# huakunyang/SummerTTS

Hardware: AMD Instinct MI355X
Metric: audio samples/sec (acoustic model + vocoder, phoneme ids -> int16 PCM on host), single_speaker_fast-shaped synthetic blob (higher is better)
Workload: dtype f32 (decoder trunk convs AND the reverse flow's WaveNet convs (wn_flow.hip, one-utterance calls): fp32 operands as 2 fp16 terms = 22-23 of their 24 mantissa bits, 3 fp16 MFMA products per fp32 product, f32 accumulation -- measured error in `parity`, same tolerance as the exact-fp32 leg; batches addi

## Files before the change

### include/summertts_hip.h

```cpp
#ifndef SUMMERTTS_HIP_H_
#define SUMMERTTS_HIP_H_

#include <stdint.h>

#ifdef __cplusplus
extern "C" {
#endif

typedef struct sts_engine sts_engine;

enum {
    STS_OK = 0,
    STS_EINVAL = -1,
    STS_EMODEL = -2,
    STS_EDEVICE = -3,
    STS_ESTATE = -4
};

int sts_create(const float* blob, int64_t blob_bytes, int device, sts_engine** out);
void sts_destroy(sts_engine* e);

int sts_speaker_num(const sts_engine* e);

typedef struct sts_model_info {
// ... 133 lines not shown

enum { STS_DBG_ATTN_BLOCK_MIN_WGS = 1,
       STS_DBG_TAIL_FUSED = 14 ,
       STS_DBG_UPS_ROWPH = 15 ,
       STS_DBG_CHAIN_STREAMS = 13 ,
       STS_DBG_H2P = 11 ,
       STS_DBG_H2P_TILE = 12 ,
       STS_DBG_MEMO_CLEAR = 10 ,
       STS_DBG_PCM_DIRECT = 9 ,
       STS_DBG_DDS_TAIL = 8 ,
       STS_DBG_ATTN_REG = 7 ,
       STS_DBG_LAUNCH_AHEAD = 6 ,
       STS_DBG_FLOW_FUSED = 5  };
enum { STS_DBG_STREAM_RETRY_STEP = 16, STS_DBG_STREAM_DIRECT = 17 };
enum { STS_DBG_POISON = 18 };
int sts_debug_set(sts_engine* e, int key, int value);

typedef struct sts_profile {
    float ms_text_encoder, ms_duration, ms_flow, ms_decoder, ms_total_device;
    float ms_decoder_mfma;
    int32_t decoder_mfma_launches;
    double flops_text_encoder, flops_duration, flops_flow, flops_decoder;
    double flops_decoder_mfma;
    double bytes_decoder_min;
    int64_t frames, samples, phonemes;
    double flops_decoder_mfma_executed;
    double bytes_text_encoder, bytes_duration, bytes_flow;
    float ms_sync_wait_host;
    double flops_decoder_bf16_issued;
    int64_t conv_math_fallbacks;
// ... 112 lines not shown
```

### summertts_amd/csrc/capi.hip

```cpp
#include <stdlib.h>
#include <string.h>

#include <algorithm>
#include <new>
#include <string>
#include <vector>

#include "engine.hpp"
#include "eq_stream.hpp"
#include "join_stream.hpp"
#include "loud_stream.hpp"

using namespace sts;

struct sts_engine { Engine eng; };

static thread_local std::string g_err;
static int set_err(int code, const std::string& s) { g_err = s; return code; }

extern "C" {

const char* sts_last_error(void) { return g_err.c_str(); }
void sts_free(void* p) { free(p); }

// ... 657 lines not shown
        case STS_DBG_ATTN_BLOCK_MIN_WGS: if (value < 1) return set_err(STS_EINVAL, "threshold must be >= 1"); e->eng.attn_block_min_wgs = value; return STS_OK;
        case STS_DBG_FLOW_FUSED: e->eng.flow_fused = value != 0; return STS_OK;
        case STS_DBG_LAUNCH_AHEAD: if (value < 0 || value > 2) return set_err(STS_EINVAL, "launch_ahead must be 0, 1 or 2"); if ((value == 2) != (e->eng.launch_ahead == 2)) { e->eng.seen_tf_.clear(); e->eng.seen_order_.clear(); } e->eng.launch_ahead = value; return STS_OK;
        case STS_DBG_H2P: e->eng.h2p = value < 0 ? 0 : (value > 4 ? 4 : value); return STS_OK;
        case STS_DBG_H2P_TILE: e->eng.h2p_tile = value; return STS_OK;
        case STS_DBG_CHAIN_STREAMS: e->eng.chain_streams_dbg = value; return STS_OK;
        case STS_DBG_TAIL_FUSED: e->eng.tail_fused = value != 0; return STS_OK;
        case STS_DBG_UPS_ROWPH: e->eng.ups_rowph = value != 0; return STS_OK;
        case STS_DBG_MEMO_CLEAR: e->eng.seen_tf_.clear(); e->eng.seen_order_.clear(); return STS_OK;
        case STS_DBG_ATTN_REG: e->eng.attn_reg = value != 0; return STS_OK;
        case STS_DBG_DDS_TAIL: e->eng.dds_tail = value != 0; return STS_OK;
        case STS_DBG_PCM_DIRECT: e->eng.pcm_direct = value != 0; return STS_OK;
        case STS_DBG_STREAM_RETRY_STEP: e->eng.stream_retry_step = value < 0 ? -1 : value; return STS_OK;
        case STS_DBG_STREAM_DIRECT: e->eng.stream_direct = value != 0; return STS_OK;
        case STS_DBG_POISON: e->eng.poison = (unsigned)value; return STS_OK;
        default: return set_err(STS_EINVAL, "unknown debug key");
    }
}
int sts_set_host_pcm(sts_engine* e, int enable) { if (!e) return set_err(STS_EINVAL, "null engine"); e->eng.host_pcm = enable != 0; return STS_OK; }
int sts_set_profiling(sts_engine* e, int enable) { if (!e) return set_err(STS_EINVAL, "null engine"); e->eng.profiling = enable == 2 ? 2 : (enable != 0 ? 1 : 0); return STS_OK; }

int sts_abi_version(void) { return STS_ABI_VERSION; }

int sts_set_output_rate(sts_engine* e, int32_t rate) {
    if (!e) return set_err(STS_EINVAL, "null engine");
    const int rc = e->eng.set_output_rate(rate);
    return rc == STS_OK ? STS_OK : set_err(rc, e->eng.error());
}
int sts_get_output_rate(const sts_engine* e) {
    if (!e) return set_err(STS_EINVAL, "null engine");
// ... 833 lines not shown
```

### summertts_amd/csrc/engine.hip

```cpp
#include "run_ctx.hpp"
#include <time.h>
#include "knobs.hpp"
#include "../../include/tts_logger.h"

#include <algorithm>
#include <chrono>
#include <math.h>
#include <stdlib.h>
#include <string.h>
#include <thread>

namespace sts {

Engine::~Engine() {
    if (stream) (void)hipStreamSynchronize(stream);
    free_model(model);
    if (arenaT_.base) (void)hipFree(arenaT_.base);
    if (arenaF_.base) (void)hipFree(arenaF_.base);
    if (pinned_) (void)hipHostFree(pinned_);
    if (pinned_pcm_) (void)hipHostFree(pinned_pcm_);
    if (d_rs_table) (void)hipFree(d_rs_table);
    if (loud_host_) (void)hipHostFree(loud_host_);
    if (lim_host_) (void)hipHostFree(lim_host_);
    if (d_eq_) (void)hipFree(d_eq_);
// ... 929 lines not shown
    size_t regA = 0, regB = 0;
    { int S = 1; for (int i = 0; i < M.n_up; i++) { S *= M.up_rate[i]; stage_elems[i] = (size_t)(3 + 4 * M.n_resk) * M.ups[i].Cout * Wcap * S;
          if (i & 1) { if (stage_elems[i] > regB) regB = stage_elems[i]; } else { if (stage_elems[i] > regA) regA = stage_elems[i]; } } }
    const long Lsb = c.Lsb = Wcap * upS + B;
    const int sbC = c.sbC = M.conv_post.Cout;
    bool use_ff = flow_fused && conv_mode == 0 && conv_math == 3 && !M.cp.empty() && wnH > 0;
    for (size_t i = 0; i < M.cp.size() && use_ff; i++)
        use_ff = M.cp[i].ff.ok && M.cp[i].wn.H == wnH && M.cp[i].wn.n == c.wnL && M.cp[i].ff.G == M.cp[0].ff.G && M.cp[i].wn.in[0].k == M.cp[0].wn.in[0].k;
    if (use_ff) {
        long tiles = 0;
        if (B == 1) tiles = (Ftot + 31) / 32;
        else for (int b = 0; b < B; b++) tiles += (p_lenF[b] + 31) / 32;
        use_ff = tiles * M.cp[0].ff.G <= 256;
    }
    c.use_ff = use_ff; c.ffG = use_ff ? M.cp[0].ff.G : 0;
    BufF& bf = c.bf;
    const OutChain& oc = c.oc;
    c.Ocap = oc.run[OS_RESAMPLE] ? out_count((long long)Wcap * hop) + B : (long long)Wcap * hop;
    if (c.join) c.Ocap = oc.run[OS_RESAMPLE] ? out_count(c.FJ * hop) + 1 : c.FJ * hop;
    const long long jwin = ss && c.join ? c.js.window_frames() * hop : c.FJ * hop;
    if (ss && c.join) c.Ocap = oc.run[OS_RESAMPLE] ? out_count(jwin) + 4 : jwin;
    if (ss && oc.run[OS_LIMIT] && oc.run[OS_RESAMPLE]) c.Ocap += B;
    pcm_in_host_ = pcm_direct && host_pcm && !ss && B == 1 && !record_taps && pinned_pcm_dev_ && (size_t)c.Ocap * 2 + 256 <= pinned_pcm_cap_ &&
                   (size_t)c.Ocap * 2 <= ((size_t)4 << 20);
    auto layoutF = [&](Arena& A) {
        A.used = 0;
        for (int q = 0; q < 2; q++) {
            bf.ff_h[q] = A.get<float>(use_ff ? (size_t)wnH * Ftot : 1);
            bf.ff_part[q] = A.get<float>(use_ff ? (size_t)c.ffG * wnH * Ftot : 1);
            bf.ff_macc[q] = A.get<float>(use_ff ? (size_t)c.ffG * (C / 2) * Ftot : 1);
// ... 105 lines not shown
            const DWn& w = cp.wn;
            const DFlowFused& ff = cp.ff;
            const int x0h = cp.flipped ? 1 : 0, x1h = 1 - x0h;
            if (pend_set >= 0 && pend_half != x0h) { finish_half(pend_half, pend_set); pend_set = -1; }
            if (w.has_cond) conv(w.cond, bt.g, lvB, bt.cond_wn, lvB, ConvOpt());
            (void)conv_args(cp.pre, nullptr, lv1, nullptr, lv1, ConvOpt(), nullptr);
            for (int l = 0; l < w.n; l++) {
                ConvOpt og; og.epi = EPI_GATE;
                (void)conv_args(w.in[l], nullptr, lv1, nullptr, lv1, og, nullptr);
                ConvOpt orr; orr.epi = EPI_RESSKIP;
                (void)conv_args(w.rs[l], nullptr, lv1, nullptr, lv1, orr, nullptr);
                FlowLayerArgs A;
                memset(&A, 0, sizeof(A));
                A.seg = lv1.seg; A.B = B; A.max_len = maxF; A.tot = Ftot;
                A.H = w.H; A.half = half; A.G = G; A.Cg = ff.Cg; A.k = w.in[l].k; A.halo = (w.in[l].k - 1) / 2;
                A.layer = l;
                if (l == 0) {
                    A.x0 = cur[x0h]; A.x0_ld = Ftot;
                    if (pend_set >= 0) {
                        A.pend = bf.ff_macc[pend_set]; A.pend_n = G; A.pend_stride = (long)hF;
                        A.x0_out = cur[x0h] == home[x0h] ? alt[x0h] : home[x0h]; A.x0_out_ld = Ftot;
                    }
                    A.w_pre = cp.pre.wh2; A.b_pre = cp.pre.bias; A.s_pre = cp.pre.h2_scale;
                    A.w_gate = ff.gate0; A.s_gate = ff.gate0_scale;
                } else {
                    A.h_in = bf.ff_h[(l - 1) & 1]; A.part_in = bf.ff_part[(l - 1) & 1]; A.part_n = G;
                    A.w_gate = w.in[l].wh2; A.s_gate = w.in[l].h2_scale;
                }
                A.part_stride = (long)((size_t)w.H * Ftot);
                A.h_out = bf.ff_h[l & 1]; A.part_out = bf.ff_part[l & 1];
                A.macc = bf.ff_macc[cs]; A.macc_stride = (long)hF; A.macc_init = l == 0;
// ... 523 lines not shown
```

### summertts_amd/csrc/engine.hpp

```cpp
#pragma once
#include <hip/hip_runtime.h>

#include <deque>
#include <map>
#include <unordered_map>
#include <string>
#include <vector>

#include "../../include/summertts_hip.h"
#include "kernels.hpp"
#include "model.hpp"

namespace sts {

struct Arena {
    char* base = nullptr; size_t cap = 0, used = 0; bool measuring = false;
    void* alloc(size_t bytes) {
        size_t a = (used + 255) & ~(size_t)255;
        used = a + bytes;
        if (measuring) return nullptr;
        return base + a;
    }
    template <typename T> T* get(size_t count) { return (T*)alloc(count * sizeof(T)); }
};
// ... 98 lines not shown
    long ahead_misses = 0;
    static constexpr size_t kMemoEntries = 1024;
    std::unordered_map<unsigned long long, long> seen_tf_; std::deque<unsigned long long> seen_order_;
    bool polite_wait = false;
    struct WaitEst { double us = 0.0; long phonemes = 0; };
    WaitEst wait_est_[2][24];
    void nap_before_wait(int which, long phonemes);
    void note_wait(int which, long phonemes, double waited_us, bool was_ready_at_wake);
    int final_sync(long phonemes);
    int ups_rowph = 1;
    int tail_fused = 1;
    int chain_streams_dbg = -1;
    int h2p = 1;
    int h2p_tile = -1;
    int flow_fused = 1;
    int stream_retry_step = -1;
    int stream_direct = 0;
    unsigned poison = 0;
    int64_t poison_bytes_ = 0;
    hipStream_t stream = nullptr;

private:
    int fail(int code, const std::string& msg) { err_ = msg; return code; }
    bool ensure(Arena& a, size_t bytes);
    bool ensure_pinned(size_t bytes);
    void poison_arena(const Arena& a);
    void poison_host16(void* p, size_t samples);
    void poison_host32(void* p, size_t words);
    ConvArgs conv_args(const DConv& c, const float* x, const Lvl& lin, float* y, const Lvl& lout, const ConvOpt& o, double* flops);
    void conv(const DConv& c, const float* x, const Lvl& lin, float* y, const Lvl& lout, const ConvOpt& o);
// ... 60 lines not shown
```

### summertts_amd/csrc/kernels.hpp

```cpp
#pragma once
#include <hip/hip_runtime.h>
#include <stdint.h>

#include <vector>

#include "../../include/summertts_hip.h"

namespace sts {

struct SegView {
    const int* off;
    const int* len;
    int scale;
    int extra;
    int ioff, ilen;
};

enum Epilogue : int {
    EPI_STORE = 0,
    EPI_RESADD = 1,
    EPI_SUB = 3,
    EPI_GATE = 4,
    EPI_RESSKIP = 5,
    EPI_TANH_PCM = 6,
// ... 84 lines not shown

struct AttnArgs {
    const float* q; const float* k; const float* v; float* o; long ld;
    const float* relk; const float* relv;
    int kc, px, win, nheads;
    SegView seg; int B, max_len;
    int block_min_wgs;
    int attn_reg;
};


struct FlowLayerArgs {
    SegView seg; int B, max_len; long tot;
    int H, half, G, Cg, k, halo;
    int layer;
    const float* x0; long x0_ld; const float* pend; int pend_n; long pend_stride; float* x0_out; long x0_out_ld;
    const void* w_pre; const float* b_pre; float s_pre;
    const float* h_in; const float* part_in; int part_n; long part_stride;
    float* h_out;
    float* part_out;
    float* macc; long macc_stride; int macc_init;
    const void* w_gate; const float* b_gate; float s_gate;
    const float* ubias; int ubias_ld;
    const void* w_c; float s_c; int rows_c, rows_res;
    const float* b_res; const float* b_m;
    unsigned* ovf;
};
struct FlowFinishArgs {
    SegView seg; int B, max_len; int half;
    const float* src; long src_ld; float* dst; long dst_ld;
    const float* macc; int n; long macc_stride;
};
bool flow_layer_shape_ok(int H, int half, int k, int dil, int n_layers);
int flow_layer_groups(int H);
void flow_layer(const FlowLayerArgs& a, hipStream_t st);
void flow_finish(const FlowFinishArgs& a, hipStream_t st);

bool conv_mfma_eligible(const ConvArgs& a);
void conv_mfma(const ConvArgs& a, hipStream_t st, int tile = -1);
constexpr int kMaxGroup = 4;
struct ConvGroup { ConvArgs g[kMaxGroup]; int n; };
struct ResLayerArgs {
    const float* x; float* y;
    const float *w1, *b1, *w2, *b2;
    int k1, dil1, k2;
    const float *wu1, *wu2;
    const void *wb1, *wb2;
    float ws1, ws2;
};
// ... 240 lines not shown
```

### summertts_amd/csrc/run_ctx.hpp

```cpp
#pragma once
#include "engine.hpp"
#include "eq_stream.hpp"
#include "loud_stream.hpp"
#include "out_chain.hpp"
#include "join_stream.hpp"

namespace sts {

#define HIPCK(call)                                                                           \
    do {                                                                                      \
        hipError_t e__ = (call);                                                              \
        if (e__ != hipSuccess) return fail(STS_EDEVICE, std::string(#call) + ": " + hipGetErrorString(e__)); \
    } while (0)

struct BufT {
    int *meta_i; float* ls; float *ns, *nsw; uint64_t* seed; int* ids; int* forced;
    float *x, *qkv, *att, *y, *x1, *ffh, *m, *logs;
    float *dh, *dt1, *dt2, *dc, *dhh, *dp29, *dr[4], *dlogw;
    int *dur, *cum, *frames;
    float *g, *cond_dp, *cond_dec, *cond_wn;
    float* plan_rate; int *plan_fixed, *plan_target; long long* plan_rem; float* dur_w;
    int* mix;
    int *gain_q, *gain_h;
    int* join_sil;
// ... 42 lines not shown
    int *pm = nullptr, *p_offT = nullptr, *p_lenT = nullptr, *p_sid = nullptr, *p_offF = nullptr, *p_lenF = nullptr, *p_one = nullptr;
    int *d_offT = nullptr, *d_lenT = nullptr, *d_sid = nullptr, *d_offF = nullptr, *d_lenF = nullptr, *d_one = nullptr, *d_win = nullptr;
    bool inl = false, no_inline_seg = false, ms = false;
    long Ftot = 0; int maxF = 0, hop = 0;
    long Fld = 0; int maxFld = 0; bool ahead = false, ahead_b = false, mapped = false, forced = false;
    bool plan = false;
    bool gain = false;
    bool join = false;
    long long FJ = 0;
    bool mix = false;
    std::vector<Engine::Noise> nz; bool any_ns = false, any_nsw = false;
    std::vector<unsigned long long> req_keys; std::vector<long> predF;
    int halo = 0; long Wcap = 0; int upS = 1; long Lsb = 0; int sbC = 0;
    long long Ocap = 0;
    bool bstream = false;
    bool use_ff = false; int ffG = 0;
    OutChain oc{}; LimiterDesign limd; int rsP = 1, rsQ = 1, eqS = 0;
    const float* stage_out(int s) const {
        const float* const o[OS_COUNT] = {bf.wave, bf.wave_gain, bf.wave_join, bf.wave_out, nullptr, bf.wave_eq, nullptr, bf.wave_lim};
        return s < 0 ? nullptr : o[s];
    }
    JsPlan js;
};
#define RUN_ALIASES(c)                                                                                                              \
    [[maybe_unused]] Model& M = model;                                                                                              \
    [[maybe_unused]] const int B = (c).B; [[maybe_unused]] const StreamSpec* const ss = (c).ss;                                     \
    [[maybe_unused]] const long Ttot = (c).Ttot; [[maybe_unused]] const int maxT = (c).maxT;                                        \
    [[maybe_unused]] const int H = (c).H, C = (c).C, FF = (c).FF, fdp = (c).fdp, wnH = (c).wnH, wnL = (c).wnL, ffn2_slices = (c).ffn2_slices; \
    [[maybe_unused]] Lvl &lvT = (c).lvT, &lvB = (c).lvB, &lv1 = (c).lv1;                                                            \
    [[maybe_unused]] BufT& bt = (c).bt; [[maybe_unused]] BufF& bf = (c).bf;                                                         \
    [[maybe_unused]] const size_t up_bytes = (c).up_bytes;                                                                          \
// ... 12 lines not shown
```

### summertts_amd/csrc/wn_flow.hip

```cpp
#include "conv_bf3_dev.hpp"

namespace sts {

#ifdef STS_TILE_TRACE
int tile_trace_bind_flow(long long* buf, unsigned capacity_records) { return tile_trace_bind(buf, capacity_records); }
#endif

constexpr int FL_WIN = 64;
constexpr int FL_NT = 32;
constexpr int FL_UR = 2;
constexpr int FL_MAXG = 8;

__device__ __forceinline__ unsigned fl_b_off(int chunk, int pos, int half, int plane, int plane_bytes) {
    return (unsigned)(chunk * 2 * plane_bytes + plane * plane_bytes + pos * 32 + ((half ^ ((pos >> 3) & 1)) << 4));
}

__device__ __forceinline__ void split4h(const float (&x)[4], unsigned (&hi)[2], unsigned (&lo)[2], float& amax) {
#pragma unroll
    for (int d = 0; d < 2; d++) {
        const f32x2 v = {x[2 * d], x[2 * d + 1]};
        const f16x2 h = __builtin_convertvector(v, f16x2);
#if STS_SPLIT_MIX
        const f32x2 v2 = v * 2048.f;
        const unsigned hu = __builtin_bit_cast(unsigned, h);
        unsigned l = 0u;
        asm("v_fma_mixlo_f16 %0, %1, %2, %3 op_sel:[0,0,0] op_sel_hi:[1,0,0]\n\t"
// ... 4 lines not shown
#else
        const f32x2 r = (v - __builtin_convertvector(h, f32x2)) * 2048.f;
        const f16x2 l = __builtin_convertvector(r, f16x2);
        hi[d] = __builtin_bit_cast(unsigned, h);
        lo[d] = __builtin_bit_cast(unsigned, l);
#endif
        amax = __builtin_fmaxf(amax, __builtin_fmaxf(__builtin_fabsf(v[0]), __builtin_fabsf(v[1])));
    }
}

constexpr int FL_WAVES = 8;
constexpr int FL_GSTEPS = 16;
template <bool L0>
__global__ __launch_bounds__(64 * FL_WAVES) __attribute__((amdgpu_waves_per_eu(2, 2))) void flow_layer_kernel(FlowLayerArgs a) {
    extern __shared__ __attribute__((aligned(16))) unsigned char fsm[];
    const int Gp = (a.G + 7) & ~7;
    const int g = (int)(blockIdx.x % (unsigned)Gp);
    if (g >= a.G) return;
    const int rest = (int)(blockIdx.x / (unsigned)Gp);
    const int ntile = (a.max_len + FL_NT - 1) / FL_NT;
    const int b = rest / ntile, tile = rest - b * ntile;
    const int len = uni(seg_len(a.seg, b));
    const int n0 = tile * FL_NT;
    if (n0 >= len) return;
    const size_t base = (size_t)uni(seg_start(a.seg, b));
    const int tid = threadIdx.x, lane = tid & 63, wave = __builtin_amdgcn_readfirstlane(tid >> 6);
    const int l31 = lane & 31, half = lane >> 5;
    const int H = a.H, hc = a.half, Cg = a.Cg, halo = a.halo;
    const int W = FL_NT + 2 * halo;
    const int NCH = H >> 4;
    const int PLANE = FL_WIN * 32;
    unsigned char* const R_h = fsm;
    unsigned char* const R_x = fsm + (size_t)NCH * 2 * PLANE;
    unsigned char* const R_a = R_x + (size_t)FL_WAVES * 4096;
    const int APL = FL_NT * 32;
    float amax = 0.f;
    constexpr int RG = 2, KS = FL_WAVES / RG;
    const int rt_l = wave % RG, kq = wave / RG;
#ifdef STS_TILE_TRACE
    long long* tt_rec = tt_open(3 + (L0 ? 1 : 0), g);
    TT_STAMP(0);
#endif

    const int nrtg = (2 * H) >> 5;
    const int c_lo = NCH * kq / KS, c_hi = NCH * (kq + 1) / KS;
    const int nsteps = (c_hi - c_lo) * a.k;
    u32x4 fa[FL_GSTEPS][1][2];
    auto gate_prefetch = [&](auto lo_c, auto hi_c) {
        constexpr int lo = decltype(lo_c)::value, hi = decltype(hi_c)::value;
        const rsrc_t wrs = make_rsrc(a.w_gate, (unsigned)((size_t)NCH * a.k * nrtg * 2048u));
        const int rt = g * RG + rt_l;
#pragma unroll
        for (int s = lo; s < hi; s++) {
            const int c = c_lo + s / a.k, j = s - (s / a.k) * a.k;
            const unsigned o = s < nsteps ? (unsigned)(((c * a.k + j) * nrtg + rt) * 2048 + lane * 16) : kOOB;
#pragma unroll
// ... 16 lines not shown
                    const unsigned off = t < ntc && cs < nkc ? (unsigned)(((g * nkc + cs) * ntc + t) * 2048 + pl * 1024 + lane * 16) : kOOB;
                    fc[ti][cs][0][pl] = __builtin_bit_cast(u32x4, __builtin_amdgcn_raw_buffer_load_b128(wrs, (int)off, 0, 0));
                }
        }
    };

    f32x4u mold[2][4];
    auto m_prefetch = [&]() {
        const rsrc_t rm = make_rsrc(a.macc + (size_t)g * a.macc_stride, a.macc_init ? 0u : (unsigned)(((size_t)a.tot * hc) * 4u));
#pragma unroll
        for (int ti = 0; ti < 2; ti++) {
            const int t = wave + FL_WAVES * ti;
#pragma unroll
            for (int q = 0; q < 4; q++) {
                const int c = t * 32 + 8 * q + 4 * half - a.rows_res;
                const bool okm = t < ntc && c >= 0 && c + 3 < hc && n0 + l31 < len;
                const unsigned off = okm ? (unsigned)(((base + (size_t)(n0 + l31)) * hc + c) * 4u) : kOOB;
                mold[ti][q] = __builtin_bit_cast(f32x4u, __builtin_amdgcn_raw_buffer_load_b128(rm, (int)off, 0, 0));
            }
        }
    };

    if constexpr (!L0) {
        gate_prefetch(I0{}, IH{});
        const int qpp = H >> 2;
        const int nunit = W * qpp;
        const unsigned span = (unsigned)(((size_t)a.tot * H) * 4u);
        const rsrc_t rh = make_rsrc(a.h_in, span);
        for (int u0 = 0; u0 < nunit; u0 += 64 * FL_WAVES * FL_UR) {
            f32x4u v[FL_UR], p[FL_UR][FL_MAXG];
            int pw[FL_UR], q4[FL_UR]; bool ok[FL_UR];
// ... 7 lines not shown
                v[r] = __builtin_bit_cast(f32x4u, __builtin_amdgcn_raw_buffer_load_b128(rh, (int)off, 0, 0));
#pragma unroll
                for (int s = 0; s < FL_MAXG; s++) {
                    const rsrc_t rp = make_rsrc(a.part_in + (size_t)s * a.part_stride, s < a.part_n ? span : 0u);
                    p[r][s] = __builtin_bit_cast(f32x4u, __builtin_amdgcn_raw_buffer_load_b128(rp, (int)off, 0, 0));
                }
            }
#pragma unroll
            for (int r = 0; r < FL_UR; r++) {
                const int u = u0 + r * 64 * FL_WAVES + tid;
                if (u >= nunit) continue;
                f32x4u s4 = v[r];
#pragma unroll
                for (int s = 0; s < FL_MAXG; s++) s4 += p[r][s];
                const int ch = q4[r] * 4;
                if (ok[r] && pw[r] >= halo && pw[r] < halo + FL_NT && ch >= g * Cg && ch < (g + 1) * Cg)
                    *(f32x4u*)(a.h_out + (base + (size_t)(n0 - halo + pw[r])) * H + ch) = s4;
                const float x4[4] = {s4[0], s4[1], s4[2], s4[3]};
                unsigned hi[2], lo[2];
                split4h(x4, hi, lo, amax);
                const int chunk = ch >> 4, hf = (ch >> 3) & 1, qd = (ch >> 2) & 1;
                unsigned char* d = R_h + fl_b_off(chunk, pw[r], hf, 0, PLANE) + qd * 8;
                *(uint2*)d = uint2{hi[0], hi[1]};
                *(uint2*)(d + PLANE) = uint2{lo[0], lo[1]};
            }
        }
        TT_STAMP(1);
        gate_prefetch(IH{}, IE{});
        c_prefetch();
        m_prefetch();
    } else {
        gate_prefetch(I0{}, IH{});
        const int nrt = H >> 5, nk = hc >> 4;
        u32x4 fp[8][1][2];
        {
            const rsrc_t wrs = make_rsrc(a.w_pre, (unsigned)((size_t)nk * nrt * 2048u));
#pragma unroll
            for (int cs = 0; cs < 8; cs++)
#pragma unroll
                for (int pl = 0; pl < 2; pl++) {
                    const unsigned o = wave < nrt && cs < nk ? (unsigned)((cs * nrt + wave) * 2048 + pl * 1024 + lane * 16) : kOOB;
                    fp[cs][0][pl] = __builtin_bit_cast(u32x4, __builtin_amdgcn_raw_buffer_load_b128(wrs, (int)o, 0, 0));
                }
        }
        const int qpp = hc >> 2;
// ... 14 lines not shown
                const unsigned off = ok[r] ? (unsigned)(((base + (size_t)pos) * hc + (size_t)q4[r] * 4) * 4u) : kOOB;
#pragma unroll
                for (int s = 0; s < FL_MAXG; s++) {
                    const rsrc_t rp = make_rsrc(a.pend + (size_t)s * a.pend_stride, s < a.pend_n ? pspan : 0u);
                    p[r][s] = __builtin_bit_cast(f32x4u, __builtin_amdgcn_raw_buffer_load_b128(rp, (int)off, 0, 0));
                }
            }
#pragma unroll
            for (int r = 0; r < FL_UR; r++) {
                const int u = u0 + r * 64 * FL_WAVES + tid;
                if (u >= nunit) continue;
                f32x4u s4 = {zv[r][0], zv[r][1], zv[r][2], zv[r][3]};
#pragma unroll
                for (int s = 0; s < FL_MAXG; s++) s4 += p[r][s];
                const int ch = q4[r] * 4;
                if (a.x0_out && ok[r] && pw[r] >= halo && pw[r] < halo + FL_NT && (q4[r] % a.G) == g) {
                    float* zp = a.x0_out + (size_t)ch * a.x0_out_ld + base + (size_t)(n0 - halo + pw[r]);
#pragma unroll
                    for (int e = 0; e < 4; e++) zp[(size_t)e * a.x0_out_ld] = s4[e];
                }
                const float x4[4] = {s4[0], s4[1], s4[2], s4[3]};
                unsigned hi[2], lo[2];
                split4h(x4, hi, lo, amax);
                const int chunk = ch >> 4, hf = (ch >> 3) & 1, qd = (ch >> 2) & 1;
                unsigned char* d = R_x + fl_b_off(chunk, pw[r], hf, 0, PLANE) + qd * 8;
                *(uint2*)d = uint2{hi[0], hi[1]};
                *(uint2*)(d + PLANE) = uint2{lo[0], lo[1]};
            }
        }
        __syncthreads();
        TT_STAMP(1);
        gate_prefetch(IH{}, IE{});
        if (wave < nrt) {
            const int rt = wave;
            f32x16 acc[1][2];
#pragma unroll
            for (int ct = 0; ct < 2; ct++)
#pragma unroll
                for (int r = 0; r < 16; r++) acc[0][ct][r] = 0.f;
#pragma unroll
            for (int cs = 0; cs < 8; cs++)
                if (cs < nk) {
                    u32x4 fb[2][2];
#pragma unroll
                    for (int ct = 0; ct < 2; ct++)
#pragma unroll
                        for (int pl = 0; pl < 2; pl++) fb[ct][pl] = *(const u32x4*)(R_x + fl_b_off(cs, ct * 32 + l31, half, pl, PLANE));
                    step_mfmas<1, 1, 2, 2, 2>(acc, fp[cs], fb);
                }
#pragma unroll
            for (int ct = 0; ct < 2; ct++) {
                const int pw_ = ct * 32 + l31;
                const int pos = n0 - halo + pw_;
                const bool inside = pos >= 0 && pos < len && pw_ < W;
#pragma unroll
                for (int hh = 0; hh < 2; hh++) {
                    float v8[8];
#pragma unroll
                    for (int e = 0; e < 8; e++) {
                        const int row = rt * 32 + hh * 16 + 8 * (e >> 2) + 4 * half + (e & 3);
                        const float t1 = acc[0][ct][hh * 8 + e] * a.s_pre + (a.b_pre ? a.b_pre[row] : 0.f);
                        v8[e] = inside ? t1 : 0.f;
                    }
                    u32x4 ph, pl;
                    split8h(v8, ph, pl, amax);
                    unsigned char* d = R_h + fl_b_off(rt * 2 + hh, pw_, half, 0, PLANE);
                    *(u32x4*)d = ph;
                    *(u32x4*)(d + PLANE) = pl;
                    if (inside && pw_ >= halo && pw_ < halo + FL_NT) {
#pragma unroll
                        for (int qd = 0; qd < 2; qd++) {
                            const int ch = rt * 32 + hh * 16 + 8 * qd + 4 * half;
                            if (ch >= g * Cg && ch < (g + 1) * Cg)
                                *(f32x4u*)(a.h_out + (base + (size_t)pos) * H + ch) = f32x4u{v8[4 * qd], v8[4 * qd + 1], v8[4 * qd + 2], v8[4 * qd + 3]};
                        }
                    }
                }
            }
        }
        c_prefetch();
        m_prefetch();
    }
    __syncthreads();
    TT_STAMP(2);
// ... 27 lines not shown
#pragma unroll
    for (int r = 0; r < 16; r++) red[((size_t)(kq * RG + rt_l) * 16 + r) * 64 + lane] = acc[0][0][r];
    __syncthreads();
    {
        const int rowb = (g * RG + rt_l) * 32;
        float gv[2];
#pragma unroll
        for (int i = 0; i < 2; i++) {
            const int r = 2 * kq + i;
            float t = 0.f, sg = 0.f;
            for (int q = 0; q < KS; q++) {
                t += red[((size_t)(q * RG + rt_l) * 16 + r) * 64 + lane];
                sg += red[((size_t)(q * RG + rt_l) * 16 + r + 8) * 64 + lane];
            }
            const int rowp = rowb + (r & 3) + 8 * (r >> 2) + 4 * half;
            t = t * a.s_gate + (a.b_gate ? a.b_gate[rowp] : 0.f);
            sg = sg * a.s_gate + (a.b_gate ? a.b_gate[rowp + 16] : 0.f);
            if (a.ubias) { t += a.ubias[(size_t)rowp * a.ubias_ld + b]; sg += a.ubias[(size_t)(rowp + 16) * a.ubias_ld + b]; }
            gv[i] = tanh_ref(t) * sigmoid_ref(sg);
        }
        const f32x2 v = {gv[0], gv[1]};
        const f16x2 hh = __builtin_convertvector(v, f16x2);
        const f32x2 rr = (v - __builtin_convertvector(hh, f32x2)) * 2048.f;
        const f16x2 ll = __builtin_convertvector(rr, f16x2);
        amax = __builtin_fmaxf(amax, __builtin_fmaxf(__builtin_fabsf(v[0]), __builtin_fabsf(v[1])));
        unsigned char* d = R_a + (size_t)rt_l * 2 * APL + l31 * 32 + ((half ^ ((l31 >> 3) & 1)) << 4) + kq * 4;
        *(unsigned*)d = __builtin_bit_cast(unsigned, hh);
        *(unsigned*)(d + APL) = __builtin_bit_cast(unsigned, ll);
    }
    __syncthreads();
    TT_STAMP(4);

    const int pos_o = n0 + l31;
    const bool col_ok = pos_o < len;
#pragma unroll
    for (int ti = 0; ti < 2; ti++) {
        const int t = wave + FL_WAVES * ti;
        if (t >= ntc) continue;
        f32x16 ac[1][1];
#pragma unroll
        for (int r = 0; r < 16; r++) ac[0][0][r] = 0.f;
#pragma unroll
        for (int cs = 0; cs < 2; cs++)
            if (cs < nkc) {
                u32x4 fb[1][2];
                const unsigned char* sp = R_a + (size_t)cs * 2 * APL + l31 * 32 + ((half ^ ((l31 >> 3) & 1)) << 4);
                fb[0][0] = *(const u32x4*)sp;
                fb[0][1] = *(const u32x4*)(sp + APL);
                step_mfmas<1, 1, 1, 2, 2>(ac, fc[ti][cs], fb);
            }
        if (!col_ok) continue;
        const int row0 = t * 32;
#pragma unroll
        for (int q = 0; q < 4; q++) {
            const int row = row0 + 8 * q + 4 * half;
            f32x4u v = {ac[0][0][4 * q] * a.s_c, ac[0][0][4 * q + 1] * a.s_c, ac[0][0][4 * q + 2] * a.s_c, ac[0][0][4 * q + 3] * a.s_c};
            if (row < a.rows_res) {
                if (g == 0 && a.b_res) v += *(const f32x4u*)(a.b_res + row);
                if (row + 3 < H) *(f32x4u*)(a.part_out + (size_t)g * a.part_stride + (base + (size_t)pos_o) * H + row) = v;
            } else {
                const int c = row - a.rows_res;
                if (c + 3 < hc) {
                    float* mp = a.macc + (size_t)g * a.macc_stride + (base + (size_t)pos_o) * hc + c;
                    if (a.macc_init) { if (g == 0 && a.b_m) v += *(const f32x4u*)(a.b_m + c); }
                    else v += mold[ti][q];
                    *(f32x4u*)mp = v;
                }
            }
        }
    }
    if (amax > kH2Limit && a.ovf) *a.ovf = 1u;
#ifdef STS_TILE_TRACE
    asm volatile("s_waitcnt vmcnt(0)" ::: "memory");
    TT_STAMP(5);
    TT_CLOSE();
#endif
}

__global__ __launch_bounds__(256) void flow_finish_kernel(FlowFinishArgs a) {
// ... 15 lines not shown
bool flow_layer_shape_ok(int H, int half, int k, int dil, int n_layers) {
    if (H < 32 || H % 32 != 0 || H > 256 || half < 16 || half % 16 != 0 || half % 4 != 0 || half > 128) return false;
    if (!(k & 1) || k < 1 || dil != 1 || (k - 1) > FL_WIN - FL_NT || n_layers < 1) return false;
    const int Cg = 32, G = H / Cg;
    if (G > FL_MAXG) return false;
    const int RG = 2, KS = FL_WAVES / RG, NCH = H / 16;
    if (((NCH + KS - 1) / KS) * k > FL_GSTEPS) return false;
    if (half / 16 > 8 || H / 32 > FL_WAVES) return false;
    const int rows_c = ((H + half) + 31) / 32 * 32;
    return rows_c / 32 <= 2 * FL_WAVES;
}
int flow_layer_groups(int H) { return H / 32; }

static size_t flow_lds_bytes(int H) {
    const size_t h = (size_t)(H / 16) * 2 * FL_WIN * 32;
    return h + (size_t)FL_WAVES * 4096 + (size_t)4 * 2 * FL_NT * 32 + 256;
}

void flow_layer(const FlowLayerArgs& a, hipStream_t st) {
    if (a.max_len <= 0 || a.B <= 0) return;
    const int Gp = (a.G + 7) & ~7;
    const int ntile = (a.max_len + FL_NT - 1) / FL_NT;
    const size_t lds = flow_lds_bytes(a.H);
    if (a.layer == 0) {
        (void)hipFuncSetAttribute((const void*)flow_layer_kernel<true>, hipFuncAttributeMaxDynamicSharedMemorySize, (int)lds);
        hipLaunchKernelGGL(flow_layer_kernel<true>, dim3((unsigned)((size_t)ntile * a.B * Gp)), dim3(64 * FL_WAVES), lds, st, a);
    } else {
        (void)hipFuncSetAttribute((const void*)flow_layer_kernel<false>, hipFuncAttributeMaxDynamicSharedMemorySize, (int)lds);
        hipLaunchKernelGGL(flow_layer_kernel<false>, dim3((unsigned)((size_t)ntile * a.B * Gp)), dim3(64 * FL_WAVES), lds, st, a);
    }
}

void flow_finish(const FlowFinishArgs& a, hipStream_t st) {
    if (a.max_len <= 0 || a.B <= 0) return;
    const long n = (long)(a.half >> 2) * a.max_len;
    hipLaunchKernelGGL(flow_finish_kernel, dim3((unsigned)((n + 255) / 256), a.B), dim3(256), 0, st, a);
}

}
```

### summertts_amd/engine.py

```python
from __future__ import annotations

import ctypes as C
import os
import subprocess
from typing import Dict, List, Optional, Sequence

import numpy as np

_HERE = os.path.dirname(os.path.abspath(__file__))
LIB_PATH = os.environ.get("SUMMERTTS_HIP_LIB") or os.path.join(_HERE, "lib", "libsummertts_hip.so")
CSRC = os.path.join(_HERE, "csrc")


def build_library(verbose: bool = False) -> str:
    subprocess.run(["make", "-C", CSRC, "-j8"], check=True, stdout=None if verbose else subprocess.DEVNULL)
    return LIB_PATH


class ModelInfo(C.Structure):
    _fields_ = [("is_multi_speaker", C.c_int32), ("lang_type", C.c_int32), ("dur_pred_type", C.c_int32),
                ("dec_type", C.c_int32), ("vocab", C.c_int32), ("hidden", C.c_int32), ("inter_channels", C.c_int32),
                ("speaker_num", C.c_int32), ("gin_channels", C.c_int32), ("samples_per_frame", C.c_int32),
                ("sample_rate", C.c_int32), ("blob_floats_consumed", C.c_int64)]

# ... 955 lines not shown
        out = np.zeros(n, LIMITER_DTYPE)
        if n:
            rc = self.lib.sts_get_limiter(self.h, out.ctypes.data, n)
            if rc < 0:
                _check(self.lib, rc)
        return out

    def set_conv_math(self, mode):
        m = {"bf16x3": 0, "f32": 1, "bf16x3_all": 2, "f16x2": 3}.get(mode, mode)
        _check(self.lib, self.lib.sts_set_conv_math(self.h, int(m)))

    def set_conv_mode(self, mode: int):
        _check(self.lib, self.lib.sts_set_conv_mode(self.h, mode))

    def debug_set(self, key: str, value: int):
        _check(self.lib, self.lib.sts_debug_set(self.h, {"attn_block_min_wgs": 1, "flow_fused": 5, "launch_ahead": 6, "attn_reg": 7, "dds_tail": 8, "pcm_direct": 9, "memo_clear": 10, "h2p": 11, "h2p_tile": 12, "chain_streams": 13, "tail_fused": 14, "ups_rowph": 15, "stream_retry_step": 16, "stream_direct": 17, "poison": 18}[key], int(value)))

    def set_profiling(self, on):
        _check(self.lib, self.lib.sts_set_profiling(self.h, 2 if on == 2 else (1 if on else 0)))

    def profile(self) -> dict:
        p = Profile()
        _check(self.lib, self.lib.sts_get_profile_ex(self.h, C.byref(p), C.sizeof(p)))
        return p.as_dict()

    def tap(self, name: str) -> np.ndarray:
        ptr = C.POINTER(C.c_float)()
        ch, ln = C.c_int32(), C.c_int64()
        _check(self.lib, self.lib.sts_get_tap(self.h, name.encode(), C.byref(ptr), C.byref(ch), C.byref(ln)))
        a = np.ctypeslib.as_array(ptr, shape=(ch.value, ln.value)).copy()
        self.lib.sts_free(ptr)
# ... 417 lines not shown
```

Baseline: 66.63 million.

## Pick adaptive flow tile width, densify grid, preload biases, set LDS attr once

Adds an adaptive time-tile width (16 or 32 columns) for the fused reverse-flow WaveNet kernel. The narrower tile is chosen when the 16-wide tile count times groups fits within the CU count, so short utterances spread across more workgroups. The launch grid drops the padding of groups to a multiple of 8, avoiding idle blocks. Bias vectors are loaded into registers early and parked in LDS so global loads leave the epilogue, and hipFuncSetAttribute is called once per device instead of every launch. The risks are extra zero-fill work for the unused LDS columns, wasted half-MFMA work at NT=16, and a larger LDS footprint.

```diff
diff --git a/include/summertts_hip.h b/include/summertts_hip.h
--- a/include/summertts_hip.h
+++ b/include/summertts_hip.h
@@ -171,6 +171,7 @@
        STS_DBG_FLOW_FUSED = 5  };
 enum { STS_DBG_STREAM_RETRY_STEP = 16, STS_DBG_STREAM_DIRECT = 17 };
 enum { STS_DBG_POISON = 18 };
+enum { STS_DBG_FLOW_TILE = 19 };
 int sts_debug_set(sts_engine* e, int key, int value);
 
 typedef struct sts_profile {
diff --git a/summertts_amd/csrc/capi.hip b/summertts_amd/csrc/capi.hip
--- a/summertts_amd/csrc/capi.hip
+++ b/summertts_amd/csrc/capi.hip
@@ -695,6 +695,7 @@
         case STS_DBG_STREAM_RETRY_STEP: e->eng.stream_retry_step = value < 0 ? -1 : value; return STS_OK;
         case STS_DBG_STREAM_DIRECT: e->eng.stream_direct = value != 0; return STS_OK;
         case STS_DBG_POISON: e->eng.poison = (unsigned)value; return STS_OK;
+        case STS_DBG_FLOW_TILE: if (value != 0 && value != 16 && value != 32) return set_err(STS_EINVAL, "flow_tile must be 0 (automatic), 16 or 32"); e->eng.flow_tile = value; return STS_OK;
         default: return set_err(STS_EINVAL, "unknown debug key");
     }
 }
diff --git a/summertts_amd/csrc/engine.hip b/summertts_amd/csrc/engine.hip
--- a/summertts_amd/csrc/engine.hip
+++ b/summertts_amd/csrc/engine.hip
@@ -967,6 +967,12 @@
         use_ff = tiles * M.cp[0].ff.G <= 256;
     }
     c.use_ff = use_ff; c.ffG = use_ff ? M.cp[0].ff.G : 0;
+    c.ff_nt = 32;
+    if (use_ff) {
+        if (cu_count_ <= 0 && (hipDeviceGetAttribute(&cu_count_, hipDeviceAttributeMultiprocessorCount, device) != hipSuccess || cu_count_ <= 0)) cu_count_ = 1;
+        const int one = (B == 1 && c.ahead && !c.predF.empty()) ? (int)c.predF[0] : p_lenF[0];
+        c.ff_nt = flow_tile_width(B == 1 ? &one : p_lenF, B, c.ffG, cu_count_, flow_tile);
+    }
     BufF& bf = c.bf;
     const OutChain& oc = c.oc;
     c.Ocap = oc.run[OS_RESAMPLE] ? out_count((long long)Wcap * hop) + B : (long long)Wcap * hop;
@@ -1102,7 +1108,7 @@
                 memset(&A, 0, sizeof(A));
                 A.seg = lv1.seg; A.B = B; A.max_len = maxF; A.tot = Ftot;
                 A.H = w.H; A.half = half; A.G = G; A.Cg = ff.Cg; A.k = w.in[l].k; A.halo = (w.in[l].k - 1) / 2;
-                A.layer = l;
+                A.layer = l; A.nt = c.ff_nt;
                 if (l == 0) {
                     A.x0 = cur[x0h]; A.x0_ld = Ftot;
                     if (pend_set >= 0) {
diff --git a/summertts_amd/csrc/engine.hpp b/summertts_amd/csrc/engine.hpp
--- a/summertts_amd/csrc/engine.hpp
+++ b/summertts_amd/csrc/engine.hpp
@@ -136,6 +136,8 @@
     int h2p = 1;
     int h2p_tile = -1;
     int flow_fused = 1;
+    int flow_tile = 0;
+    int cu_count_ = 0;
     int stream_retry_step = -1;
     int stream_direct = 0;
     unsigned poison = 0;
diff --git a/summertts_amd/csrc/flow_tile.hpp b/summertts_amd/csrc/flow_tile.hpp
--- /dev/null
+++ b/summertts_amd/csrc/flow_tile.hpp
@@ -0,0 +1,12 @@
+#pragma once
+
+namespace sts {
+
+inline int flow_tile_rule(const int* len, int B, int G, int cus, int forced) {
+    if (forced == 16 || forced == 32) return forced;
+    long long t16 = 0;
+    for (int b = 0; b < B; b++) t16 += len[b] > 0 ? (len[b] + 15) / 16 : 0;
+    return t16 * G <= (long long)cus ? 16 : 32;
+}
+
+}
diff --git a/summertts_amd/csrc/kernels.hpp b/summertts_amd/csrc/kernels.hpp
--- a/summertts_amd/csrc/kernels.hpp
+++ b/summertts_amd/csrc/kernels.hpp
@@ -122,6 +122,8 @@
     SegView seg; int B, max_len; long tot;
     int H, half, G, Cg, k, halo;
     int layer;
+    int nt;
+    int dense;
     const float* x0; long x0_ld; const float* pend; int pend_n; long pend_stride; float* x0_out; long x0_out_ld;
     const void* w_pre; const float* b_pre; float s_pre;
     const float* h_in; const float* part_in; int part_n; long part_stride;
@@ -141,6 +143,7 @@
 };
 bool flow_layer_shape_ok(int H, int half, int k, int dil, int n_layers);
 int flow_layer_groups(int H);
+int flow_tile_width(const int* len, int B, int G, int cus, int forced);
 void flow_layer(const FlowLayerArgs& a, hipStream_t st);
 void flow_finish(const FlowFinishArgs& a, hipStream_t st);
 
diff --git a/summertts_amd/csrc/run_ctx.hpp b/summertts_amd/csrc/run_ctx.hpp
--- a/summertts_amd/csrc/run_ctx.hpp
+++ b/summertts_amd/csrc/run_ctx.hpp
@@ -80,7 +80,7 @@
     int halo = 0; long Wcap = 0; int upS = 1; long Lsb = 0; int sbC = 0;
     long long Ocap = 0;
     bool bstream = false;
-    bool use_ff = false; int ffG = 0;
+    bool use_ff = false; int ffG = 0; int ff_nt = 32;
     OutChain oc{}; LimiterDesign limd; int rsP = 1, rsQ = 1, eqS = 0;
     const float* stage_out(int s) const {
         const float* const o[OS_COUNT] = {bf.wave, bf.wave_gain, bf.wave_join, bf.wave_out, nullptr, bf.wave_eq, nullptr, bf.wave_lim};
diff --git a/summertts_amd/csrc/wn_flow.hip b/summertts_amd/csrc/wn_flow.hip
--- a/summertts_amd/csrc/wn_flow.hip
+++ b/summertts_amd/csrc/wn_flow.hip
@@ -1,4 +1,13 @@
 #include "conv_bf3_dev.hpp"
+#include "flow_tile.hpp"
+#include <atomic>
+
+#ifndef STS_FLOW_OPS_EARLY
+#define STS_FLOW_OPS_EARLY 1
+#endif
+#ifndef STS_FLOW_DENSE32
+#define STS_FLOW_DENSE32 1
+#endif
 
 namespace sts {
 
@@ -10,6 +19,7 @@
 constexpr int FL_NT = 32;
 constexpr int FL_UR = 2;
 constexpr int FL_MAXG = 8;
+constexpr int FL_SB_GATE = 0, FL_SB_U = 64, FL_SB_PRE = 128, FL_SB_RES = 384, FL_SB_M = 640, FL_SB_FLOATS = 768;
 
 __device__ __forceinline__ unsigned fl_b_off(int chunk, int pos, int half, int plane, int plane_bytes) {
     return (unsigned)(chunk * 2 * plane_bytes + plane * plane_bytes + pos * 32 + ((half ^ ((pos >> 3) & 1)) << 4));
@@ -44,25 +54,28 @@
 template <bool L0>
 __global__ __launch_bounds__(64 * FL_WAVES) __attribute__((amdgpu_waves_per_eu(2, 2))) void flow_layer_kernel(FlowLayerArgs a) {
     extern __shared__ __attribute__((aligned(16))) unsigned char fsm[];
-    const int Gp = (a.G + 7) & ~7;
+    const int Gp = a.dense ? a.G : (a.G + 7) & ~7;
     const int g = (int)(blockIdx.x % (unsigned)Gp);
     if (g >= a.G) return;
     const int rest = (int)(blockIdx.x / (unsigned)Gp);
-    const int ntile = (a.max_len + FL_NT - 1) / FL_NT;
+    const int NT = a.nt;
+    const int ntile = (a.max_len + NT - 1) / NT;
     const int b = rest / ntile, tile = rest - b * ntile;
     const int len = uni(seg_len(a.seg, b));
-    const int n0 = tile * FL_NT;
+    const int n0 = tile * NT;
     if (n0 >= len) return;
     const size_t base = (size_t)uni(seg_start(a.seg, b));
     const int tid = threadIdx.x, lane = tid & 63, wave = __builtin_amdgcn_readfirstlane(tid >> 6);
     const int l31 = lane & 31, half = lane >> 5;
     const int H = a.H, hc = a.half, Cg = a.Cg, halo = a.halo;
-    const int W = FL_NT + 2 * halo;
+    const int W = NT + 2 * halo;
+    const int WF = FL_NT + 2 * halo;
     const int NCH = H >> 4;
     const int PLANE = FL_WIN * 32;
     unsigned char* const R_h = fsm;
     unsigned char* const R_x = fsm + (size_t)NCH * 2 * PLANE;
     unsigned char* const R_a = R_x + (size_t)FL_WAVES * 4096;
+    [[maybe_unused]] float* const sbias = (float*)(R_a + (size_t)4 * 2 * FL_NT * 32);
     const int APL = FL_NT * 32;
     float amax = 0.f;
     constexpr int RG = 2, KS = FL_WAVES / RG;
@@ -70,6 +83,28 @@
 #ifdef STS_TILE_TRACE
     long long* tt_rec = tt_open(3 + (L0 ? 1 : 0), g);
     TT_STAMP(0);
+#endif
+
+#if STS_FLOW_OPS_EARLY
+    const int rowg0 = g * RG * 32;
+    float bq_gate = 0.f, bq_u = 0.f, bq_pre = 0.f, bq_res = 0.f, bq_m = 0.f;
+    if (tid < 64) {
+        if (a.b_gate) bq_gate = a.b_gate[rowg0 + tid];
+        if (a.ubias) bq_u = a.ubias[(size_t)(rowg0 + tid) * a.ubias_ld + b];
+    } else if (tid < 64 + 128) {
+        if (g == 0 && a.macc_init && a.b_m && tid - 64 < hc) bq_m = a.b_m[tid - 64];
+    }
+    if (tid < 256) {
+        if (L0 && a.b_pre && tid < H) bq_pre = a.b_pre[tid];
+    } else {
+        if (g == 0 && a.b_res && tid - 256 < a.rows_res) bq_res = a.b_res[tid - 256];
+    }
+    auto bias_park = [&]() {
+        if (tid < 64) { sbias[FL_SB_GATE + tid] = bq_gate; sbias[FL_SB_U + tid] = bq_u; }
+        else if (tid < 64 + 128) sbias[FL_SB_M + tid - 64] = bq_m;
+        if (tid < 256) { if (L0) sbias[FL_SB_PRE + tid] = bq_pre; }
+        else sbias[FL_SB_RES + tid - 256] = bq_res;
+    };
 #endif
 
     const int nrtg = (2 * H) >> 5;
@@ -116,7 +151,7 @@
 #pragma unroll
             for (int q = 0; q < 4; q++) {
                 const int c = t * 32 + 8 * q + 4 * half - a.rows_res;
-                const bool okm = t < ntc && c >= 0 && c + 3 < hc && n0 + l31 < len;
+                const bool okm = t < ntc && c >= 0 && c + 3 < hc && l31 < NT && n0 + l31 < len;
                 const unsigned off = okm ? (unsigned)(((base + (size_t)(n0 + l31)) * hc + c) * 4u) : kOOB;
                 mold[ti][q] = __builtin_bit_cast(f32x4u, __builtin_amdgcn_raw_buffer_load_b128(rm, (int)off, 0, 0));
             }
@@ -154,7 +189,7 @@
 #pragma unroll
                 for (int s = 0; s < FL_MAXG; s++) s4 += p[r][s];
                 const int ch = q4[r] * 4;
-                if (ok[r] && pw[r] >= halo && pw[r] < halo + FL_NT && ch >= g * Cg && ch < (g + 1) * Cg)
+                if (ok[r] && pw[r] >= halo && pw[r] < halo + NT && ch >= g * Cg && ch < (g + 1) * Cg)
                     *(f32x4u*)(a.h_out + (base + (size_t)(n0 - halo + pw[r])) * H + ch) = s4;
                 const float x4[4] = {s4[0], s4[1], s4[2], s4[3]};
                 unsigned hi[2], lo[2];
@@ -165,10 +200,19 @@
                 *(uint2*)(d + PLANE) = uint2{lo[0], lo[1]};
             }
         }
+        for (int u = nunit + tid; u < WF * qpp; u += 64 * FL_WAVES) {
+            const int pz = u / qpp, ch = (u - pz * qpp) * 4;
+            unsigned char* d = R_h + fl_b_off(ch >> 4, pz, (ch >> 3) & 1, 0, PLANE) + ((ch >> 2) & 1) * 8;
+            *(uint2*)d = uint2{0u, 0u};
+            *(uint2*)(d + PLANE) = uint2{0u, 0u};
+        }
         TT_STAMP(1);
         gate_prefetch(IH{}, IE{});
         c_prefetch();
         m_prefetch();
+#if STS_FLOW_OPS_EARLY
+        bias_park();
+#endif
     } else {
         gate_prefetch(I0{}, IH{});
         const int nrt = H >> 5, nk = hc >> 4;
@@ -213,7 +257,7 @@
 #pragma unroll
                 for (int s = 0; s < FL_MAXG; s++) s4 += p[r][s];
                 const int ch = q4[r] * 4;
-                if (a.x0_out && ok[r] && pw[r] >= halo && pw[r] < halo + FL_NT && (q4[r] % a.G) == g) {
+                if (a.x0_out && ok[r] && pw[r] >= halo && pw[r] < halo + NT && (q4[r] % a.G) == g) {
                     float* zp = a.x0_out + (size_t)ch * a.x0_out_ld + base + (size_t)(n0 - halo + pw[r]);
 #pragma unroll
                     for (int e = 0; e < 4; e++) zp[(size_t)e * a.x0_out_ld] = s4[e];
@@ -227,25 +271,36 @@
                 *(uint2*)(d + PLANE) = uint2{lo[0], lo[1]};
             }
         }
+        const int nct = (W + 31) >> 5;
+        for (int u = nunit + tid; u < nct * 32 * qpp; u += 64 * FL_WAVES) {
+            const int uu = u - nunit, k4 = uu / (nct * 32 - W), pz = W + uu - k4 * (nct * 32 - W), ch = k4 * 4;
+            unsigned char* d = R_x + fl_b_off(ch >> 4, pz, (ch >> 3) & 1, 0, PLANE) + ((ch >> 2) & 1) * 8;
+            *(uint2*)d = uint2{0u, 0u};
+            *(uint2*)(d + PLANE) = uint2{0u, 0u};
+        }
+#if STS_FLOW_OPS_EARLY
+        bias_park();
+#endif
         __syncthreads();
         TT_STAMP(1);
         gate_prefetch(IH{}, IE{});
         if (wave < nrt) {
             const int rt = wave;
-            f32x16 acc[1][2];
+            f32x16 acc[2][1][1];
 #pragma unroll
             for (int ct = 0; ct < 2; ct++)
 #pragma unroll
-                for (int r = 0; r < 16; r++) acc[0][ct][r] = 0.f;
+                for (int r = 0; r < 16; r++) acc[ct][0][0][r] = 0.f;
 #pragma unroll
             for (int cs = 0; cs < 8; cs++)
                 if (cs < nk) {
-                    u32x4 fb[2][2];
+                    u32x4 fb[2][1][2];
 #pragma unroll
                     for (int ct = 0; ct < 2; ct++)
 #pragma unroll
-                        for (int pl = 0; pl < 2; pl++) fb[ct][pl] = *(const u32x4*)(R_x + fl_b_off(cs, ct * 32 + l31, half, pl, PLANE));
-                    step_mfmas<1, 1, 2, 2, 2>(acc, fp[cs], fb);
+                        for (int pl = 0; pl < 2; pl++) fb[ct][0][pl] = *(const u32x4*)(R_x + fl_b_off(cs, ct * 32 + l31, half, pl, PLANE));
+                    step_mfmas<1, 1, 1, 2, 2>(acc[0], fp[cs], fb[0]);
+                    if (nct > 1) step_mfmas<1, 1, 1, 2, 2>(acc[1], fp[cs], fb[1]);
                 }
 #pragma unroll
             for (int ct = 0; ct < 2; ct++) {
@@ -258,7 +313,11 @@
 #pragma unroll
                     for (int e = 0; e < 8; e++) {
                         const int row = rt * 32 + hh * 16 + 8 * (e >> 2) + 4 * half + (e & 3);
-                        const float t1 = acc[0][ct][hh * 8 + e] * a.s_pre + (a.b_pre ? a.b_pre[row] : 0.f);
+#if STS_FLOW_OPS_EARLY
+                        const float t1 = acc[ct][0][0][hh * 8 + e] * a.s_pre + sbias[FL_SB_PRE + row];
+#else
+                        const float t1 = acc[ct][0][0][hh * 8 + e] * a.s_pre + (a.b_pre ? a.b_pre[row] : 0.f);
+#endif
                         v8[e] = inside ? t1 : 0.f;
                     }
                     u32x4 ph, pl;
@@ -266,7 +325,7 @@
                     unsigned char* d = R_h + fl_b_off(rt * 2 + hh, pw_, half, 0, PLANE);
                     *(u32x4*)d = ph;
                     *(u32x4*)(d + PLANE) = pl;
-                    if (inside && pw_ >= halo && pw_ < halo + FL_NT) {
+                    if (inside && pw_ >= halo && pw_ < halo + NT) {
 #pragma unroll
                         for (int qd = 0; qd < 2; qd++) {
                             const int ch = rt * 32 + hh * 16 + 8 * qd + 4 * half;
@@ -324,9 +383,16 @@
                 sg += red[((size_t)(q * RG + rt_l) * 16 + r + 8) * 64 + lane];
             }
             const int rowp = rowb + (r & 3) + 8 * (r >> 2) + 4 * half;
+#if STS_FLOW_OPS_EARLY
+            const int rl = rowp - rowg0;
+            t = t * a.s_gate + sbias[FL_SB_GATE + rl];
+            sg = sg * a.s_gate + sbias[FL_SB_GATE + rl + 16];
+            if (a.ubias) { t += sbias[FL_SB_U + rl]; sg += sbias[FL_SB_U + rl + 16]; }
+#else
             t = t * a.s_gate + (a.b_gate ? a.b_gate[rowp] : 0.f);
             sg = sg * a.s_gate + (a.b_gate ? a.b_gate[rowp + 16] : 0.f);
             if (a.ubias) { t += a.ubias[(size_t)rowp * a.ubias_ld + b]; sg += a.ubias[(size_t)(rowp + 16) * a.ubias_ld + b]; }
+#endif
             gv[i] = tanh_ref(t) * sigmoid_ref(sg);
         }
         const f32x2 v = {gv[0], gv[1]};
@@ -342,7 +408,7 @@
     TT_STAMP(4);
 
     const int pos_o = n0 + l31;
-    const bool col_ok = pos_o < len;
+    const bool col_ok = l31 < NT && pos_o < len;
 #pragma unroll
     for (int ti = 0; ti < 2; ti++) {
         const int t = wave + FL_WAVES * ti;
@@ -366,13 +432,21 @@
             const int row = row0 + 8 * q + 4 * half;
             f32x4u v = {ac[0][0][4 * q] * a.s_c, ac[0][0][4 * q + 1] * a.s_c, ac[0][0][4 * q + 2] * a.s_c, ac[0][0][4 * q + 3] * a.s_c};
             if (row < a.rows_res) {
+#if STS_FLOW_OPS_EARLY
+                if (g == 0 && a.b_res) v += *(const f32x4u*)(sbias + FL_SB_RES + row);
+#else
                 if (g == 0 && a.b_res) v += *(const f32x4u*)(a.b_res + row);
+#endif
                 if (row + 3 < H) *(f32x4u*)(a.part_out + (size_t)g * a.part_stride + (base + (size_t)pos_o) * H + row) = v;
             } else {
                 const int c = row - a.rows_res;
                 if (c + 3 < hc) {
                     float* mp = a.macc + (size_t)g * a.macc_stride + (base + (size_t)pos_o) * hc + c;
+#if STS_FLOW_OPS_EARLY
+                    if (a.macc_init) { if (g == 0 && a.b_m) v += *(const f32x4u*)(sbias + FL_SB_M + c); }
+#else
                     if (a.macc_init) { if (g == 0 && a.b_m) v += *(const f32x4u*)(a.b_m + c); }
+#endif
                     else v += mold[ti][q];
                     *(f32x4u*)mp = v;
                 }
@@ -418,19 +492,39 @@
 
 static size_t flow_lds_bytes(int H) {
     const size_t h = (size_t)(H / 16) * 2 * FL_WIN * 32;
-    return h + (size_t)FL_WAVES * 4096 + (size_t)4 * 2 * FL_NT * 32 + 256;
-}
-
-void flow_layer(const FlowLayerArgs& a, hipStream_t st) {
-    if (a.max_len <= 0 || a.B <= 0) return;
-    const int Gp = (a.G + 7) & ~7;
-    const int ntile = (a.max_len + FL_NT - 1) / FL_NT;
+    return h + (size_t)FL_WAVES * 4096 + (size_t)4 * 2 * FL_NT * 32 + (size_t)FL_SB_FLOATS * 4 + 256;
+}
+
+int flow_tile_width(const int* len, int B, int G, int cus, int forced) {
+#ifdef STS_FLOW_TILE_FORCE
+    if (forced == 0) forced = STS_FLOW_TILE_FORCE;
+#endif
+    return flow_tile_rule(len, B, G, cus, forced);
+}
+
+template <bool L0>
+static void flow_lds_attr_once() {
+    static std::atomic<unsigned long long> done{0ull};
+    int dev = 0;
+    if (hipGetDevice(&dev) != hipSuccess) dev = 64;
+    if (dev >= 0 && dev < 64 && (done.load(std::memory_order_acquire) >> dev & 1ull)) return;
+    (void)hipFuncSetAttribute((const void*)flow_layer_kernel<L0>, hipFuncAttributeMaxDynamicSharedMemorySize, (int)flow_lds_bytes(256));
+    if (dev >= 0 && dev < 64) done.fetch_or(1ull << dev, std::memory_order_release);
+}
+
+void flow_layer(const FlowLayerArgs& a0, hipStream_t st) {
+    if (a0.max_len <= 0 || a0.B <= 0) return;
+    FlowLayerArgs a = a0;
+    if (a.nt != 16) a.nt = FL_NT;
+    a.dense = (a.nt == 16 || STS_FLOW_DENSE32) ? 1 : 0;
+    const int Gp = a.dense ? a.G : (a.G + 7) & ~7;
+    const int ntile = (a.max_len + a.nt - 1) / a.nt;
     const size_t lds = flow_lds_bytes(a.H);
     if (a.layer == 0) {
-        (void)hipFuncSetAttribute((const void*)flow_layer_kernel<true>, hipFuncAttributeMaxDynamicSharedMemorySize, (int)lds);
+        flow_lds_attr_once<true>();
         hipLaunchKernelGGL(flow_layer_kernel<true>, dim3((unsigned)((size_t)ntile * a.B * Gp)), dim3(64 * FL_WAVES), lds, st, a);
     } else {
-        (void)hipFuncSetAttribute((const void*)flow_layer_kernel<false>, hipFuncAttributeMaxDynamicSharedMemorySize, (int)lds);
+        flow_lds_attr_once<false>();
         hipLaunchKernelGGL(flow_layer_kernel<false>, dim3((unsigned)((size_t)ntile * a.B * Gp)), dim3(64 * FL_WAVES), lds, st, a);
     }
 }
diff --git a/summertts_amd/engine.py b/summertts_amd/engine.py
--- a/summertts_amd/engine.py
+++ b/summertts_amd/engine.py
@@ -993,7 +993,7 @@
         _check(self.lib, self.lib.sts_set_conv_mode(self.h, mode))
 
     def debug_set(self, key: str, value: int):
-        _check(self.lib, self.lib.sts_debug_set(self.h, {"attn_block_min_wgs": 1, "flow_fused": 5, "launch_ahead": 6, "attn_reg": 7, "dds_tail": 8, "pcm_direct": 9, "memo_clear": 10, "h2p": 11, "h2p_tile": 12, "chain_streams": 13, "tail_fused": 14, "ups_rowph": 15, "stream_retry_step": 16, "stream_direct": 17, "poison": 18}[key], int(value)))
+        _check(self.lib, self.lib.sts_debug_set(self.h, {"attn_block_min_wgs": 1, "flow_fused": 5, "launch_ahead": 6, "attn_reg": 7, "dds_tail": 8, "pcm_direct": 9, "memo_clear": 10, "h2p": 11, "h2p_tile": 12, "chain_streams": 13, "tail_fused": 14, "ups_rowph": 15, "stream_retry_step": 16, "stream_direct": 17, "poison": 18, "flow_tile": 19}[key], int(value)))
 
     def set_profiling(self, on):
         _check(self.lib, self.lib.sts_set_profiling(self.h, 2 if on == 2 else (1 if on else 0)))
```

Result: no change. 67.29 million, median of 6 (+1.0%).
